# tomoyoshki/focal

Hardware: AMD Instinct MI355X
Metric: pretrain windows/sec (whole node), FOCAL SW_Transformer (higher is better)
Workload: dtype bf16

## Files before the change

focal_amd/csrc/gemm_dw_group.hpp:

```cpp
#pragma once
#include "gemm_pipe.hpp"

constexpr int DWG_MAX_PROBLEMS = FOCAL_DW_GROUP_MAX_PROBLEMS;

struct DwGroupProblem {
  const bf16_t* A; const bf16_t* B; float* C; float* colsum;
  int lda, ldb, ldc;
  int M, N, rows;
  int splits;
  int exclusive;
};
struct DwGroupParams {
  int nprob;
  int wg_end[DWG_MAX_PROBLEMS];
  DwGroupProblem prob[DWG_MAX_PROBLEMS];
};

template <int RPS, int NST>
__global__ __launch_bounds__(512) void focal_dw_group_kernel(const DwGroupParams gp) {
  constexpr int SUB_BYTES = RPS * 128;
  constexpr int STAGE_BYTES = 4 * SUB_BYTES;
  constexpr int PPS = RPS / 8;
  constexpr int LPW = 4 * PPS / 8;
  static_assert(RPS % 32 == 0 && (4 * PPS) % 8 == 0, "stage geometry");
  constexpr int NFA = 4, NFB = 2;
  constexpr int WPITCH = 32 + 4;
  static_assert(NST * STAGE_BYTES >= 8 * 16 * WPITCH * 4, "epilogue staging must fit in the ring");
  extern __shared__ __attribute__((aligned(1024))) char dwg_lds[];
  const int tid = threadIdx.x, lane = tid & 63, g = lane >> 4, l15 = lane & 15, tq = l15 >> 2, tp = l15 & 3;
  const int wave = __builtin_amdgcn_readfirstlane(tid >> 6);
  const int wm = wave >> 2, wn = wave & 3;

  const int logical = xcd_remap(blockIdx.x, gridDim.x);
  int pi = 0;
#pragma unroll
  for (int q = 0; q < DWG_MAX_PROBLEMS - 1; ++q) pi += (q < gp.nprob - 1 && logical >= gp.wg_end[q]) ? 1 : 0;
  const DwGroupProblem& p = gp.prob[pi];
  const int local = logical - (pi > 0 ? gp.wg_end[pi - 1] : 0);
  const int tiles_n = p.N >> 7, ntiles = (p.M >> 7) * tiles_n;
  const int tile = local % ntiles, sp = local / ntiles;
  const int m0 = (tile / tiles_n) << 7, n0 = (tile % tiles_n) << 7;
  const int KT = p.rows / RPS;
  const int kt_per = (KT + p.splits - 1) / p.splits;
  const int kt0 = min(KT, sp * kt_per), kt1 = min(KT, kt0 + kt_per);
  const int nk = kt1 - kt0;

  auto swz = [](int r) { return (((r >> 1) & 1) << 1) | (((r >> 3) & 1) << 2); };

  uint32_t goff[LPW];
  const char* gbase[LPW];
  long gstep[LPW];
#pragma unroll
  for (int t = 0; t < LPW; ++t) {
    const int q = wave + 8 * t;
    const int sub = q / PPS, row = 8 * (q % PPS) + (lane >> 3), pos = lane & 7;
    const int chunk = pos ^ swz(row);
    if (sub < 2) {
      goff[t] = (uint32_t)(((long)row * p.lda + m0 + 64 * sub + chunk * 8) * 2);
      gbase[t] = reinterpret_cast<const char*>(p.A);
      gstep[t] = (long)RPS * p.lda * 2;
    } else {
      goff[t] = (uint32_t)(((long)row * p.ldb + n0 + 64 * (sub - 2) + chunk * 8) * 2);
      gbase[t] = reinterpret_cast<const char*>(p.B);
      gstep[t] = (long)RPS * p.ldb * 2;
    }
  }
  auto fill = [&](int kt, int stage) {
#pragma unroll
    for (int t = 0; t < LPW; ++t) {
      const int q = wave + 8 * t;
      char* dst = dwg_lds + stage * STAGE_BYTES + q * 1024;
      __builtin_amdgcn_global_load_lds((pipe_glb_ptr)(gbase[t] + (long)kt * gstep[t] + goff[t]), (pipe_lds_ptr)dst, 16, 0, 0);
    }
  };

  f32x4 acc[NFA][NFB], accb[NFA];
#pragma unroll
  for (int i = 0; i < NFA; ++i) {
    accb[i] = f32x4{0.f, 0.f, 0.f, 0.f};
#pragma unroll
    for (int j = 0; j < NFB; ++j) acc[i][j] = f32x4{0.f, 0.f, 0.f, 0.f};
  }
  const bool do_bias = (p.colsum != nullptr) && (n0 == 0) && (wn == 0);
  bf16x8 ones;
#pragma unroll
  for (int e = 0; e < 8; ++e) ones[e] = (bf16_t)1.0f;

  const int row_lo = 8 * g + tq;
  const int sw = swz(row_lo);
  int fr_a[NFA], fr_b[NFB];
#pragma unroll
  for (int i = 0; i < NFA; ++i) fr_a[i] = wm * SUB_BYTES + row_lo * 128 + (((2 * i + (tp >> 1)) ^ sw) << 4) + (tp & 1) * 8;
#pragma unroll
  for (int j = 0; j < NFB; ++j)
    fr_b[j] = (2 + (wn >> 1)) * SUB_BYTES + row_lo * 128 + (((2 * (2 * (wn & 1) + j) + (tp >> 1)) ^ sw) << 4) + (tp & 1) * 8;
  const uint32_t lds0 = pipe_lds_addr(dwg_lds);
  auto compute = [&](int stage) {
    const uint32_t sb = lds0 + stage * STAGE_BYTES;
    pipe_static_for<0, RPS / 32>([&](auto kc) {
      constexpr int KO = decltype(kc)::value * 32 * 128;
      bf16x4 al[NFA], ah[NFA], bl[NFB], bh[NFB];
#pragma unroll
      for (int i = 0; i < NFA; ++i) {
        al[i] = pipe_lds_read_tr<KO>(sb + fr_a[i]);
        ah[i] = pipe_lds_read_tr<KO + 4 * 128>(sb + fr_a[i]);
      }
#pragma unroll
      for (int j = 0; j < NFB; ++j) {
        bl[j] = pipe_lds_read_tr<KO>(sb + fr_b[j]);
        bh[j] = pipe_lds_read_tr<KO + 4 * 128>(sb + fr_b[j]);
      }
      bf16x8 xa[NFA], wb[NFB];
#pragma unroll
      for (int i = 0; i < NFA; ++i) xa[i] = __builtin_shufflevector(al[i], ah[i], 0, 1, 2, 3, 4, 5, 6, 7);
#pragma unroll
      for (int j = 0; j < NFB; ++j) wb[j] = __builtin_shufflevector(bl[j], bh[j], 0, 1, 2, 3, 4, 5, 6, 7);
      pipe_lds_wait(xa, wb);
#pragma unroll
      for (int i = 0; i < NFA; ++i)
#pragma unroll
        for (int j = 0; j < NFB; ++j) acc[i][j] = mma16(wb[j], xa[i], acc[i][j]);
      if (do_bias) {
#pragma unroll
        for (int i = 0; i < NFA; ++i) accb[i] = mma16(ones, xa[i], accb[i]);
      }
    });
  };

#pragma unroll
  for (int s = 0; s < NST - 1; ++s)
    if (s < nk) fill(kt0 + s, s);
  int stage = 0, fstage = NST - 1;
  for (int i = 0; i < nk; ++i) {
    const int ahead = nk - 1 - i;
    if (NST >= 4 && ahead >= 2) pipe_wait_barrier<2 * LPW>();
    else if (NST >= 3 && ahead >= 1) pipe_wait_barrier<LPW>();
    else pipe_wait_barrier<0>();
    if (i + NST - 1 < nk) fill(kt0 + i + NST - 1, fstage);
    compute(stage);
    stage = (stage + 1 == NST) ? 0 : stage + 1;
    fstage = (fstage + 1 == NST) ? 0 : fstage + 1;
  }
  if (nk == 0) return;
#if defined(DWG_LAB_NOEPI)
  {
    float lab = 0.f;
#pragma unroll
    for (int i = 0; i < NFA; ++i) {
      lab += accb[i][0];
#pragma unroll
      for (int j = 0; j < NFB; ++j) lab += acc[i][j][0] + acc[i][j][1] + acc[i][j][2] + acc[i][j][3];
    }
    if (lab == 12345.678f) p.C[0] = 1.f;
    return;
  }
#endif

  const int mrow = m0 + 64 * wm, ncol = n0 + 32 * wn;
  if (p.splits == 1 && p.exclusive) {
#pragma unroll
    for (int i = 0; i < NFA; ++i)
#pragma unroll
      for (int j = 0; j < NFB; ++j) {
        float4* dst = reinterpret_cast<float4*>(p.C + (long)(mrow + 16 * i + l15) * p.ldc + ncol + 16 * j + 4 * g);
        float4 v = *dst;
        v.x += acc[i][j][0]; v.y += acc[i][j][1]; v.z += acc[i][j][2]; v.w += acc[i][j][3];
        *dst = v;
      }
  } else {
    asm volatile("s_barrier" ::: "memory");
    float* est = reinterpret_cast<float*>(dwg_lds) + wave * 16 * WPITCH;
    const int ecol = lane & 31, erow = lane >> 5;
#pragma unroll
    for (int i = 0; i < NFA; ++i) {
#pragma unroll
      for (int j = 0; j < NFB; ++j)
        *reinterpret_cast<float4*>(est + l15 * WPITCH + j * 16 + g * 4) = make_float4(acc[i][j][0], acc[i][j][1], acc[i][j][2], acc[i][j][3]);
      asm volatile("s_waitcnt lgkmcnt(0)" ::: "memory");
      float* crow = p.C + (long)(mrow + 16 * i + erow) * p.ldc + ncol + ecol;
#pragma unroll 4
#if defined(DWG_LAB_STORE)
      for (int r = 0; r < 16; r += 2) crow[(long)r * p.ldc] = est[(r + erow) * WPITCH + ecol];
#else
      for (int r = 0; r < 16; r += 2) atomicAdd(crow + (long)r * p.ldc, est[(r + erow) * WPITCH + ecol]);
#endif
      asm volatile("s_waitcnt lgkmcnt(0)" ::: "memory");
    }
  }
  if (do_bias && g == 0) {
#pragma unroll
    for (int i = 0; i < NFA; ++i) atomicAdd(p.colsum + mrow + 16 * i + l15, accb[i][0]);
  }
}

template <int RPS>
static inline int focal_dw_group_plan(DwGroupParams& gp, int target_wgs, int min_steps) {
  long work = 0;
  for (int q = 0; q < gp.nprob; ++q) work += (long)(gp.prob[q].M >> 7) * (gp.prob[q].N >> 7) * (gp.prob[q].rows / RPS);
  long per = (work + target_wgs - 1) / target_wgs;
  if (per < min_steps) per = min_steps;
  int total = 0;
  for (int it = 0; it < 64; ++it) {
    total = 0;
    for (int q = 0; q < gp.nprob; ++q) {
      DwGroupProblem& p = gp.prob[q];
      const int KT = p.rows / RPS;
      int s = (int)((KT + per - 1) / per);
      if (s < 1) s = 1;
      p.splits = s;
      total += (p.M >> 7) * (p.N >> 7) * s;
    }
    bool can_shrink = false;
    for (int q = 0; q < gp.nprob; ++q) can_shrink = can_shrink || gp.prob[q].splits > 1;
    if (total <= target_wgs || !can_shrink) break;
    per += (per + 15) / 16;
  }
  int end = 0;
  for (int q = 0; q < gp.nprob; ++q) {
    end += (gp.prob[q].M >> 7) * (gp.prob[q].N >> 7) * gp.prob[q].splits;
    gp.wg_end[q] = end;
  }
  for (int q = gp.nprob; q < DWG_MAX_PROBLEMS; ++q) gp.wg_end[q] = end;
  return end;
}

template <int RPS, int NST>
static inline hipError_t focal_launch_dw_group(const DwGroupParams& gp, int wgs, hipStream_t stream) {
  constexpr int LDS_BYTES = NST * 4 * RPS * 128;
  auto kern = focal_dw_group_kernel<RPS, NST>;
  static std::atomic<bool> attr_set{false};
  if (!attr_set.load(std::memory_order_acquire)) {
    hipError_t e = hipFuncSetAttribute(reinterpret_cast<const void*>(kern), hipFuncAttributeMaxDynamicSharedMemorySize, LDS_BYTES);
    if (e != hipSuccess) return e;
    attr_set.store(true, std::memory_order_release);
  }
  FOCAL_LAUNCH(kern, dim3(wgs), dim3(512), LDS_BYTES, stream, gp);
  return hipGetLastError();
}
```

focal_amd/csrc/linear.hip:

```cpp
#include <stdlib.h>
#include "gemm.hpp"
#include "gemm_dw_group.hpp"
#include "gemm_dw_ring.hpp"
#include "gemm_ring.hpp"

static MaskParams to_mask(const focal_drop_desc& d, int ncols) {
  MaskParams m;
  m.seed = d.rng;
  m.stream_elem = d.stream_elem;
  m.p_elem = d.p_elem;
  m.stream_path = d.stream_path;
  m.p_path = d.p_path;
  m.rows_per_sample = d.rows_per_sample;
  m.ncols = ncols;
  return m;
}
static MaskParams no_mask() {
  MaskParams m;
  memset(&m, 0, sizeof(m));
  return m;
}

static int check_desc(const focal_linear_desc* d) {
  FOCAL_CHECK_ARG(d != nullptr, "linear: null descriptor");
// ... 134 lines not shown
  p.proB = no_mask();
  focal_drop_desc dd;
  memset(&dd, 0, sizeof(dd));
  if (mask) dd = *mask;
  p.epi = to_mask(dd, d->K);
  hipError_t e;
  if (d->K == 64 && d->M >= 4096 && !focal_ring_disabled() &&
      focal_ring_fits<float, EPI_LN_BWD, true, 128, 64, 6, true, 8, 1, 2, false>(p)) {
    focal_note_kernel("focal_gemm_ring_kernel<f32, epi=%d (LayerNorm backward), trB=1, 128x64, 8x1 waves, ring 6, panel resident>", EPI_LN_BWD);
    e = focal_launch_gemm_ring<float, EPI_LN_BWD, true, 128, 64, 6, true, 8, 1, 2, false>(p, (hipStream_t)stream);
  } else if (d->K == 128 && d->M >= 4096 && !focal_ring_disabled() &&
             focal_ring_fits<float, EPI_LN_BWD, true, 64, 128, 4, false, 4, 1, 2, false, false>(p)) {
    focal_note_kernel("focal_gemm_ring_kernel<f32, epi=%d (LayerNorm backward), trB=1, 64x128, 4x1 waves, ring 4>", EPI_LN_BWD);
    e = focal_launch_gemm_ring<float, EPI_LN_BWD, true, 64, 128, 4, false, 4, 1, 2, false, false>(p, (hipStream_t)stream);
  } else if (d->K == 256 && d->M >= 2048 && !focal_ring_disabled() && getenv("FOCAL_LAB_LN_BWD_RING256") != nullptr &&
             focal_ring_fits<float, EPI_LN_BWD, true, 64, 256, 2, false, 4, 1, 2, false, false>(p)) {
    focal_note_kernel("focal_gemm_ring_kernel<f32, epi=%d (LayerNorm backward), trB=1, 64x256, 4x1 waves, ring 2>", EPI_LN_BWD);
    e = focal_launch_gemm_ring<float, EPI_LN_BWD, true, 64, 256, 2, false, 4, 1, 2, false, false>(p, (hipStream_t)stream);
  } else {
    focal_note_kernel("focal_gemm_pipe_kernel<f32, epi=%d (LayerNorm backward), trB=1, %dx%d, 4x%d waves>", EPI_LN_BWD, d->K == 256 ? 64 : 128,
                      d->K, d->K == 256 ? 2 : 1);
    e = d->K == 64    ? focal_launch_gemm_pipe<float, EPI_LN_BWD, true, 128, 64, 2, 4, 1>(p, (hipStream_t)stream)
        : d->K == 128 ? focal_launch_gemm_pipe<float, EPI_LN_BWD, true, 128, 128, 2, 4, 1>(p, (hipStream_t)stream)
                      : focal_launch_gemm_pipe<float, EPI_LN_BWD, true, 64, 256, 2, 4, 2>(p, (hipStream_t)stream);
  }
  if (e != hipSuccess) {
    focal_set_error("linear_bwd_data_ln: launch failed: %s", hipGetErrorString(e));
    return FOCAL_EHIP;
  }
  return FOCAL_OK;
}

extern "C" int focal_linear_bwd_weight(const focal_linear_desc* d, const void* dy, const void* x, float* dw, float* dbias,
                                       void* stream) {
  if (int rc = check_desc(d)) return rc;
  FOCAL_CHECK_ARG(dy && x && dw, "linear_bwd_weight: null tensor");
  GemmSpec s;
  s.compute = d->dtype;
  s.a_dtype = d->y_dtype; s.b_dtype = d->x_dtype; s.c_dtype = FOCAL_F32;
  s.tra = true; s.trb = true;
  const bool masked = d->epilogue == FOCAL_EPI_RESIDUAL || (d->y_dtype == FOCAL_F32 && d->x_dtype != FOCAL_F32);
  s.proA = masked ? PRO_MASK : PRO_NONE;
  s.proB = PRO_NONE;
  s.epi = EPI_ATOMIC;
  GemmParams p;
  memset(&p, 0, sizeof(p));
  p.M = d->N; p.N = d->K; p.K = d->M;
  p.A = dy; p.lda = d->N;
  p.B = x; p.ldb = d->K;
  p.C = dw; p.ldc = d->K;
  p.batch = 1; p.alpha = 1.f;
  p.splits = 1;
  p.dw_target = d->dw_workgroups;
  p.proA = masked ? to_mask(d->out_drop, d->N) : no_mask();
  p.proB = no_mask();
  p.epi = no_mask();
  p.colsumA = dbias;
  return focal_launch_gemm(s, p, (hipStream_t)stream);
}

static bool dw_launch_plan(const focal_linear_desc* d, int* kernel, int* wgs) {
  if (check_desc(d) != FOCAL_OK) return false;
  int bm, bn, splits;
  focal_dw_plan(d->N, d->K, d->M, d->dw_workgroups, &bm, &bn, &splits);
  const bool masked = d->epilogue == FOCAL_EPI_RESIDUAL || (d->y_dtype == FOCAL_F32 && d->x_dtype != FOCAL_F32);
  const bool ring = d->dtype == FOCAL_BF16 && d->x_dtype == FOCAL_BF16 && d->y_dtype == FOCAL_BF16 && !masked && bm == 64 && bn == 64 &&
                    focal_dw_ring_shape(d->N, d->K, d->M);
  *kernel = ring ? 2 : 1;
  if (ring && splits >= 2) splits = focal_dw_ring_pairs(d->N, d->K, splits);
  *wgs = ((d->N + bm - 1) / bm) * ((d->K + bn - 1) / bn) * splits;
  return true;
}

extern "C" int focal_linear_bwd_weight_workgroups(const focal_linear_desc* d) {
  int kernel, wgs;
  return dw_launch_plan(d, &kernel, &wgs) ? wgs : 0;
}

extern "C" int focal_linear_bwd_weight_kernel(const focal_linear_desc* d) {
  int kernel, wgs;
  return dw_launch_plan(d, &kernel, &wgs) ? kernel : 0;
}

static bool dw_group_fits(const focal_dw_problem& q) {
  return q.M > 0 && q.N > 0 && q.K > 0 && q.M % 64 == 0 && q.N % 128 == 0 && q.K % 128 == 0 && q.dy && q.x && q.dw &&
         ((uintptr_t)q.dy % 16 == 0) && ((uintptr_t)q.x % 16 == 0) && ((uintptr_t)q.dw % 16 == 0);
}

extern "C" int focal_linear_bwd_weight_group_supported(int dtype, int M, int N, int K) {
  return dtype == FOCAL_BF16 && M > 0 && M % 64 == 0 && N % 128 == 0 && K % 128 == 0;
}

static int dw_group_build(int dtype, int n, const focal_dw_problem* probs, DwGroupParams* gp, int* wgs) {
  FOCAL_CHECK_ARG(dtype == FOCAL_BF16, "linear_bwd_weight_group: bf16 operands only (dtype %d)", dtype);
  FOCAL_CHECK_ARG(n >= 1 && n <= DWG_MAX_PROBLEMS && probs, "linear_bwd_weight_group: 1 .. %d problems (got %d)", DWG_MAX_PROBLEMS, n);
  memset(gp, 0, sizeof(*gp));
  gp->nprob = n;
  for (int i = 0; i < n; ++i) {
    const focal_dw_problem& q = probs[i];
    FOCAL_CHECK_ARG(dw_group_fits(q), "linear_bwd_weight_group: problem %d (M=%d N=%d K=%d) needs M %% 64 == 0, N, K %% 128 == 0 and 16-byte aligned tensors", i, q.M, q.N, q.K);
    DwGroupProblem& p = gp->prob[i];
    p.A = reinterpret_cast<const bf16_t*>(q.dy); p.lda = q.N;
    p.B = reinterpret_cast<const bf16_t*>(q.x); p.ldb = q.K;
    p.C = q.dw; p.ldc = q.K;
    p.colsum = q.dbias;
    p.M = q.N; p.N = q.K; p.rows = q.M;
    p.exclusive = q.exclusive ? 1 : 0;
  }
  const int target = getenv("FOCAL_LAB_DWG_TARGET") ? atoi(getenv("FOCAL_LAB_DWG_TARGET")) : 256, min_steps = 8;
  *wgs = focal_dw_group_plan<64>(*gp, target, min_steps);
  return FOCAL_OK;
}

static bool dw_ring_group_fits(const focal_dw_problem& q) {
  return q.M >= 64 && q.M % 64 == 0 && q.N > 0 && q.N % 64 == 0 && q.K > 0 && q.K % 64 == 0 && q.dy && q.x && q.dw &&
         ((uintptr_t)q.dy % 16 == 0) && ((uintptr_t)q.x % 16 == 0);
}
static bool dw_group_uses_ring(int n, const focal_dw_problem* probs) {
  if (!probs || n < 1 || n > DWR_MAX_PROBLEMS) return false;
  bool all128 = true, all64 = true;
  for (int i = 0; i < n; ++i) { all128 = all128 && dw_group_fits(probs[i]); all64 = all64 && dw_ring_group_fits(probs[i]); }
  return !all128 && all64;
}
static int dw_ring_group_build(int dtype, int n, const focal_dw_problem* probs, DwRingGroupParams* gp, int* wgs) {
  FOCAL_CHECK_ARG(dtype == FOCAL_BF16, "linear_bwd_weight_group: bf16 operands only (dtype %d)", dtype);
  memset(gp, 0, sizeof(*gp));
  gp->nprob = n;
  for (int i = 0; i < n; ++i) {
    const focal_dw_problem& q = probs[i];
    GemmParams& p = gp->prob[i];
    p.M = q.N; p.N = q.K; p.K = q.M;
    p.A = q.dy; p.lda = q.N;
    p.B = q.x; p.ldb = q.K;
    p.C = q.dw; p.ldc = q.K;
    p.batch = 1; p.alpha = 1.f; p.splits = 1;
    p.colsumA = q.dbias;
  }
  *wgs = focal_dw_ring_group_plan<2>(*gp);
  return FOCAL_OK;
}

extern "C" int focal_linear_bwd_weight_group_kind(int dtype, int M, int N, int K) {
  if (dtype != FOCAL_BF16 || M <= 0 || M % 64 != 0) return 0;
  if (N % 128 == 0 && K % 128 == 0) return 2;
  return (N > 0 && K > 0 && N % 64 == 0 && K % 64 == 0) ? 1 : 0;
}

extern "C" int focal_linear_bwd_weight_group(int dtype, int n, const focal_dw_problem* probs, void* stream) {
  if (dw_group_uses_ring(n, probs)) {
    DwRingGroupParams rp;
    int rw = 0;
    if (int rc = dw_ring_group_build(dtype, n, probs, &rp, &rw)) return rc;
    focal_note_kernel("focal_dw_ring_group_kernel<64, 4, 2>");
    hipError_t e = focal_launch_dw_ring_group<64, 4, 2>(rp, rw, (hipStream_t)stream);
    if (e != hipSuccess) {
      focal_set_error("linear_bwd_weight_group (64-tile ring): launch failed: %s", hipGetErrorString(e));
      return FOCAL_EHIP;
    }
    return FOCAL_OK;
  }
  DwGroupParams gp;
  int wgs = 0;
  if (int rc = dw_group_build(dtype, n, probs, &gp, &wgs)) return rc;
  hipError_t e = focal_launch_dw_group<64, 4>(gp, wgs, (hipStream_t)stream);
  if (e != hipSuccess) {
    focal_set_error("linear_bwd_weight_group: launch failed: %s", hipGetErrorString(e));
    return FOCAL_EHIP;
  }
  return FOCAL_OK;
}

static int dw_tail_build(int compute, int n, const focal_dw_problem* probs, int workgroups, DwTailGroup* g) {
  FOCAL_CHECK_ARG(compute == FOCAL_BF16 || compute == FOCAL_F32, "linear_bwd_weight_group_f32: bad compute dtype %d", compute);
  FOCAL_CHECK_ARG(n >= 1 && n <= DW_TAIL_MAX && probs, "linear_bwd_weight_group_f32: 1 .. %d problems (got %d)", DW_TAIL_MAX, n);
  memset(g, 0, sizeof(*g));
  g->n = n;
  const int target = (workgroups > 0 ? workgroups : 1024) / n;
  int end = 0;
  for (int i = 0; i < n; ++i) {
    const focal_dw_problem& q = probs[i];
    FOCAL_CHECK_ARG(q.dy && q.x && q.dw && q.M > 0 && q.N > 0 && q.K > 0, "linear_bwd_weight_group_f32: problem %d: null tensor or empty shape", i);
    GemmParams& p = g->p[i];
    p.M = q.N; p.N = q.K; p.K = q.M;
    p.A = q.dy; p.lda = q.N;
    p.B = q.x; p.ldb = q.K;
    p.C = q.dw; p.ldc = q.K;
    p.batch = 1; p.alpha = 1.f;
    p.colsumA = q.dbias;
    int bm, bn, splits;
    focal_dw_plan(p.M, p.N, q.M, target < 1 ? 1 : target, &bm, &bn, &splits);
    p.splits = splits;
    end += ((p.M + bm - 1) / bm) * ((p.N + bn - 1) / bn) * splits;
    g->wg_end[i] = end;
  }
// ... 24 lines not shown
```

focal_amd/ops.py:

```python
import ctypes as C
import math
import os

import torch

from . import _lib
from ._lib import (ACT_GELU, ACT_NONE, ACT_RELU_OUT, EPI_GELU, EPI_NONE, EPI_RELU, EPI_RESIDUAL, FOCAL_BF16, FOCAL_F32,
                   AdamWDesc, AttnDesc, BNDesc, ConvDesc, ConvInDesc, DropDesc, Embed2Desc, EmbedDesc, FFTDesc, GRUDesc, LinearDesc,
                   LNDesc, LossDesc, MlpDesc, check)

_TORCH2CODE = {torch.float32: FOCAL_F32, torch.bfloat16: FOCAL_BF16}
_CODE2TORCH = {v: k for k, v in _TORCH2CODE.items()}


def code(dtype):
    return _TORCH2CODE[dtype]


def torch_dtype(c):
    return _CODE2TORCH[c]


def _stream():
    return torch.cuda.current_stream().cuda_stream
# ... 444 lines not shown
    out = torch.empty(rows, Cc, dtype=dtype, device=g.device)
    check(_lib.load().focal_mask_cast(code(dtype), rows, Cc, _p(g), C.byref(mask or NO_DROP), _p(out), _stream()))
    return out


def linear_desc(dtype_code, M, N, K, x_dtype, y_dtype, act_in=ACT_NONE, epilogue=EPI_NONE, splits=1, out_drop=None, dw_workgroups=0):
    return LinearDesc(dtype_code, M, N, K, x_dtype, y_dtype, act_in, epilogue, splits, out_drop or NO_DROP, dw_workgroups)


def linear_fwd(d, x, w, bias, resid, y, act_grad=None):
    check(_lib.load().focal_linear_fwd(C.byref(d), _p(x), _p(w), _p(bias), _p(resid), _p(y), _p(act_grad), _stream()))


def linear_resid_ln_fwd(d, x, w, bias, resid, y, gamma, beta, out_dtype, eps=1e-5):
    y_ln = torch.empty(d.M, d.N, dtype=out_dtype, device=y.device)
    stats = torch.empty(d.M, 2, dtype=torch.float32, device=y.device)
    check(_lib.load().focal_linear_resid_ln_fwd(C.byref(d), _p(x), _p(w), _p(bias), _p(resid), _p(y), _p(gamma), _p(beta), eps,
                                                _p(y_ln), _p(stats), _stream()))
    return y_ln, stats


def resid_ln_supported(dtype_code, N, K):
    return bool(_lib.load().focal_linear_resid_ln_supported(dtype_code, N, K))


def linear_bwd_data(d, dy, w, x, dx):
    check(_lib.load().focal_linear_bwd_data(C.byref(d), _p(dy), _p(w), _p(x), _p(dx), _stream()))


def bwd_data_ln_supported(dtype_code, N, K):
    return bool(_lib.load().focal_linear_bwd_data_ln_supported(dtype_code, N, K))


def linear_bwd_data_ln(d, dy, w, ln_x, ln_stats, ln_gamma, g, dgamma, dbeta, g_masked=None, mask=None):
    _need_cuda(dy, w, ln_x, ln_stats, ln_gamma, g, dgamma, dbeta, g_masked)
    if g_masked is not None:
        mask = mask or NO_DROP
    check(_lib.load().focal_linear_bwd_data_ln(C.byref(d), _p(dy), _p(w), _p(ln_x), _p(ln_stats), _p(ln_gamma), _p(g), _p(dgamma), _p(dbeta),
                                               _p(g_masked), C.byref(mask) if mask is not None else None, _stream()))


def linear_bwd_weight(d, dy, x, dw, dbias):
    check(_lib.load().focal_linear_bwd_weight(C.byref(d), _p(dy), _p(x), _p(dw), _p(dbias), _stream()))


def dw_group_supported(dtype_code, M, N, K):
    return bool(_lib.load().focal_linear_bwd_weight_group_supported(dtype_code, M, N, K))


def dw_group_kind(dtype_code, M, N, K):
    return int(_lib.load().focal_linear_bwd_weight_group_kind(dtype_code, M, N, K))


def _dw_problems(items, exclusive):
    arr = (_lib.DwProblem * len(items))()
    for i, (dy, x, dw, db) in enumerate(items):
        _need_cuda(dy, x, dw, db)
        arr[i] = _lib.DwProblem(_p(dy), _p(x), _p(dw), _p(db), dy.shape[0], dy.shape[1], x.shape[1], 1 if exclusive else 0)
    return arr


DW_GROUP_MAX_PROBLEMS = 20


def linear_bwd_weight_group(dtype_code, items, exclusive=True):
    arr = _dw_problems(items, exclusive)
    check(_lib.load().focal_linear_bwd_weight_group(dtype_code, len(items), arr, _stream()))


DW_TAIL_MAX = 8


def linear_bwd_weight_group_f32(compute_code, items, workgroups=0):
    for dy, x, dw, db in items:
        if dy.dtype != torch.float32 or x.dtype != torch.float32 or dy.dim() != 2 or x.dim() != 2 or not (dy.is_contiguous() and x.is_contiguous()):
            raise _lib.FocalHipError("linear_bwd_weight_group_f32: dy and x must be contiguous fp32 matrices")
    check(_lib.load().focal_linear_bwd_weight_group_f32(compute_code, len(items), _dw_problems(items, False), workgroups, _stream()))


def linear_bwd_weight_group_workgroups(dtype_code, items, exclusive=True):
    return _lib.load().focal_linear_bwd_weight_group_workgroups(dtype_code, len(items), _dw_problems(items, exclusive))


def linear(x, w, bias=None, *, compute, y_dtype=None, resid=None, act_in=ACT_NONE, epilogue=EPI_NONE, splits=1,
           out_drop=None, act_grad=None):
    _need_cuda(x, w, bias, resid)
    M, K = x.shape
    N = w.shape[0]
    y_dtype = y_dtype or compute
    d = linear_desc(code(compute), M, N, K, code(x.dtype), code(y_dtype), act_in, epilogue, splits, out_drop)
    y = (torch.zeros if splits > 1 else torch.empty)(M, N, dtype=y_dtype, device=x.device)
    linear_fwd(d, x, w, bias, resid, y, act_grad)
    return y, d


def mlp_supported(dtype, Cc, hidden):
    return bool(_lib.load().focal_mlp_supported(code(dtype), Cc, hidden))


def mlp_desc(dtype_code, M, Cc, hidden, drop_hidden=None, drop_out=None, ln_eps=1e-5):
    return MlpDesc(dtype_code, M, Cc, hidden, drop_hidden or NO_DROP, drop_out or NO_DROP, ln_eps)


def mlp_mask_bits(d, device):
    if d.drop_hidden.p_elem <= 0.0:
        return None
    return torch.empty(d.M, 8, dtype=torch.int32, device=device)


def _next_ln(d, like, next_ln):
    if next_ln is None:
        return (None,) * 4, None
    y_ln = torch.empty(d.M, d.C, dtype=like.dtype, device=like.device)
    stats = torch.empty(d.M, 2, dtype=torch.float32, device=like.device)
    return (_p(next_ln[0]), _p(next_ln[1]), _p(y_ln), _p(stats)), (y_ln, stats)


def _ln_mask(ln, key):
    return None if ln is None else C.byref(ln.get(key) or NO_DROP)


def mlp_fwd(d, a, resid, w1, b1, w2, b2, y, next_ln=None, mask_bits=None):
    _need_cuda(a, resid, w1, b1, w2, b2, y, mask_bits)
    ln_ptrs, out = _next_ln(d, a, next_ln)
    check(_lib.load().focal_mlp_fwd(C.byref(d), _p(a), _p(resid), _p(w1), _p(b1), _p(w2), _p(b2), _p(y), *ln_ptrs, _p(mask_bits), _stream()))
    return out


def mlp_proj_supported(dtype, Cc, hidden):
    return bool(_lib.load().focal_mlp_proj_supported(code(dtype), Cc, hidden))


def mlp_proj_fwd(d, o, x, wp, bp, drop_proj, g2, bt2, x_mid, w1, b1, w2, b2, y, next_ln=None, mask_bits=None):
    _need_cuda(o, x, wp, bp, g2, bt2, x_mid, w1, b1, w2, b2, y, mask_bits)
    a2 = torch.empty(d.M, d.C, dtype=o.dtype, device=o.device)
    st2 = torch.empty(d.M, 2, dtype=torch.float32, device=o.device)
    mask = drop_proj or NO_DROP
    ln_ptrs, out = _next_ln(d, o, next_ln)
    check(_lib.load().focal_mlp_proj_fwd(C.byref(d), _p(o), _p(x), _p(wp), _p(bp), C.byref(mask), _p(g2), _p(bt2), _p(x_mid), _p(a2), _p(st2), _p(w1), _p(b1),
                                         _p(w2), _p(b2), _p(y), *ln_ptrs, _p(mask_bits), _stream()))
    return (a2, st2), out


def mlp_wide_supported(dtype, Cc, hidden):
    return bool(_lib.load().focal_mlp_wide_supported(code(dtype), Cc, hidden))


def mlp_wide_fwd(d, a, resid, w1, b1, w2, b2, y, h, hg, next_ln=None):
    _need_cuda(a, resid, w1, b1, w2, b2, y, h, hg)
    assert h.shape == (d.M, d.hidden) and hg.shape == h.shape and h.dtype == a.dtype and hg.dtype == a.dtype and h.is_contiguous() and hg.is_contiguous()
    ln_ptrs, out = _next_ln(d, a, next_ln)
    check(_lib.load().focal_mlp_wide_fwd(C.byref(d), _p(a), _p(resid), _p(w1), _p(b1), _p(w2), _p(b2), _p(y), _p(h), _p(hg), *ln_ptrs, _stream()))
    return out


def mlp_wide_proj_supported(dtype, Cc, hidden):
    return bool(_lib.load().focal_mlp_wide_proj_supported(code(dtype), Cc, hidden))


def mlp_wide_proj_fwd(d, o, x, wp, bp, drop_proj, g2, bt2, x_mid, w1, b1, w2, b2, y, h, hg, next_ln=None):
    _need_cuda(o, x, wp, bp, g2, bt2, x_mid, w1, b1, w2, b2, y, h, hg)
    a2 = torch.empty(d.M, d.C, dtype=o.dtype, device=o.device)
    st2 = torch.empty(d.M, 2, dtype=torch.float32, device=o.device)
    mask = drop_proj or NO_DROP
    ln_ptrs, out = _next_ln(d, o, next_ln)
    check(_lib.load().focal_mlp_wide_proj_fwd(C.byref(d), _p(o), _p(x), _p(wp), _p(bp), C.byref(mask), _p(g2), _p(bt2), _p(x_mid), _p(a2), _p(st2), _p(w1), _p(b1),
# ... 477 lines not shown
```

Measured before the change: 52580.

## Balance grouped weight-gradient GEMM work with a stream-K style unit split

Replaces the per-problem split-K planner of the grouped dW kernel with a work-unit scheduler. Each workgroup can now walk several (tile, k-range) segments in a loop, so the total (tile, stage) units are spread evenly across workgroups. A host-side cost model picks between this balanced cut and the old sliced cut, and memoizes the choice per shape. The epilogue now stages the whole 64x32 wave tile at once and rotates the atomic row order by segment key to spread atomic contention. The balanced cut adds per-segment atomic flushes and barriers in exchange for less tail imbalance.

```diff
diff --git a/focal_amd/csrc/gemm_dw_group.hpp b/focal_amd/csrc/gemm_dw_group.hpp
--- a/focal_amd/csrc/gemm_dw_group.hpp
+++ b/focal_amd/csrc/gemm_dw_group.hpp
@@ -1,4 +1,5 @@
 #pragma once
+#include <climits>
 #include "gemm_pipe.hpp"
 
 constexpr int DWG_MAX_PROBLEMS = FOCAL_DW_GROUP_MAX_PROBLEMS;
@@ -7,14 +8,51 @@
   const bf16_t* A; const bf16_t* B; float* C; float* colsum;
   int lda, ldb, ldc;
   int M, N, rows;
-  int splits;
+  int band, nfull;
   int exclusive;
 };
 struct DwGroupParams {
   int nprob;
-  int wg_end[DWG_MAX_PROBLEMS];
+  int pieces;
+  int share, extra;
+  int chunk_end[2 * DWG_MAX_PROBLEMS];
   DwGroupProblem prob[DWG_MAX_PROBLEMS];
 };
+static_assert(sizeof(DwGroupParams) <= 4096, "the kernel-argument struct must stay within what a launch accepts");
+
+struct DwGroupSeg {
+  int prob, tile, kt0, nk;
+  int adv;
+  int key;
+  int whole;
+};
+
+template <int RPS>
+__host__ __device__ __forceinline__ DwGroupSeg focal_dw_group_locate(const DwGroupParams& gp, int u, int u1) {
+  int ci = 0, start = 0;
+#pragma unroll
+  for (int q = 0; q < 2 * DWG_MAX_PROBLEMS - 1; ++q) {
+    const int e = gp.chunk_end[q];
+    if (u >= e) { ci = q + 1; start = e; }
+  }
+  const bool rem = ci >= gp.nprob;
+  DwGroupSeg s;
+  s.prob = rem ? ci - gp.nprob : ci;
+  const DwGroupProblem& p = gp.prob[s.prob];
+  const int ntiles = (p.M >> 7) * (p.N >> 7), KT = p.rows / RPS;
+  const int base = p.nfull * p.band;
+  const int len = rem ? KT - base : p.band;
+  const int local = u - start;
+  const int piece = gp.pieces ? local : local / len, within = gp.pieces ? 0 : local - piece * len;
+  const int bandi = rem ? p.nfull : piece / ntiles;
+  s.tile = rem ? piece : piece - bandi * ntiles;
+  s.kt0 = (rem ? base : bandi * p.band) + within;
+  s.nk = (gp.pieces || len - within < u1 - u) ? len - within : u1 - u;
+  s.adv = gp.pieces ? 1 : s.nk;
+  s.key = 2 * bandi + (within != 0 ? 1 : 0);
+  s.whole = (s.kt0 == 0 && s.nk == KT) ? 1 : 0;
+  return s;
+}
 
 template <int RPS, int NST>
 __global__ __launch_bounds__(512) void focal_dw_group_kernel(const DwGroupParams gp) {
@@ -25,66 +63,13 @@
   static_assert(RPS % 32 == 0 && (4 * PPS) % 8 == 0, "stage geometry");
   constexpr int NFA = 4, NFB = 2;
   constexpr int WPITCH = 32 + 4;
-  static_assert(NST * STAGE_BYTES >= 8 * 16 * WPITCH * 4, "epilogue staging must fit in the ring");
+  static_assert(NST * STAGE_BYTES >= 8 * 64 * WPITCH * 4, "epilogue staging (a wave's 64 x 32 outputs, eight waves) must fit in the ring");
   extern __shared__ __attribute__((aligned(1024))) char dwg_lds[];
   const int tid = threadIdx.x, lane = tid & 63, g = lane >> 4, l15 = lane & 15, tq = l15 >> 2, tp = l15 & 3;
   const int wave = __builtin_amdgcn_readfirstlane(tid >> 6);
   const int wm = wave >> 2, wn = wave & 3;
 
-  const int logical = xcd_remap(blockIdx.x, gridDim.x);
-  int pi = 0;
-#pragma unroll
-  for (int q = 0; q < DWG_MAX_PROBLEMS - 1; ++q) pi += (q < gp.nprob - 1 && logical >= gp.wg_end[q]) ? 1 : 0;
-  const DwGroupProblem& p = gp.prob[pi];
-  const int local = logical - (pi > 0 ? gp.wg_end[pi - 1] : 0);
-  const int tiles_n = p.N >> 7, ntiles = (p.M >> 7) * tiles_n;
-  const int tile = local % ntiles, sp = local / ntiles;
-  const int m0 = (tile / tiles_n) << 7, n0 = (tile % tiles_n) << 7;
-  const int KT = p.rows / RPS;
-  const int kt_per = (KT + p.splits - 1) / p.splits;
-  const int kt0 = min(KT, sp * kt_per), kt1 = min(KT, kt0 + kt_per);
-  const int nk = kt1 - kt0;
-
   auto swz = [](int r) { return (((r >> 1) & 1) << 1) | (((r >> 3) & 1) << 2); };
-
-  uint32_t goff[LPW];
-  const char* gbase[LPW];
-  long gstep[LPW];
-#pragma unroll
-  for (int t = 0; t < LPW; ++t) {
-    const int q = wave + 8 * t;
-    const int sub = q / PPS, row = 8 * (q % PPS) + (lane >> 3), pos = lane & 7;
-    const int chunk = pos ^ swz(row);
-    if (sub < 2) {
-      goff[t] = (uint32_t)(((long)row * p.lda + m0 + 64 * sub + chunk * 8) * 2);
-      gbase[t] = reinterpret_cast<const char*>(p.A);
-      gstep[t] = (long)RPS * p.lda * 2;
-    } else {
-      goff[t] = (uint32_t)(((long)row * p.ldb + n0 + 64 * (sub - 2) + chunk * 8) * 2);
-      gbase[t] = reinterpret_cast<const char*>(p.B);
-      gstep[t] = (long)RPS * p.ldb * 2;
-    }
-  }
-  auto fill = [&](int kt, int stage) {
-#pragma unroll
-    for (int t = 0; t < LPW; ++t) {
-      const int q = wave + 8 * t;
-      char* dst = dwg_lds + stage * STAGE_BYTES + q * 1024;
-      __builtin_amdgcn_global_load_lds((pipe_glb_ptr)(gbase[t] + (long)kt * gstep[t] + goff[t]), (pipe_lds_ptr)dst, 16, 0, 0);
-    }
-  };
-
-  f32x4 acc[NFA][NFB], accb[NFA];
-#pragma unroll
-  for (int i = 0; i < NFA; ++i) {
-    accb[i] = f32x4{0.f, 0.f, 0.f, 0.f};
-#pragma unroll
-    for (int j = 0; j < NFB; ++j) acc[i][j] = f32x4{0.f, 0.f, 0.f, 0.f};
-  }
-  const bool do_bias = (p.colsum != nullptr) && (n0 == 0) && (wn == 0);
-  bf16x8 ones;
-#pragma unroll
-  for (int e = 0; e < 8; ++e) ones[e] = (bf16_t)1.0f;
 
   const int row_lo = 8 * g + tq;
   const int sw = swz(row_lo);
@@ -95,133 +80,293 @@
   for (int j = 0; j < NFB; ++j)
     fr_b[j] = (2 + (wn >> 1)) * SUB_BYTES + row_lo * 128 + (((2 * (2 * (wn & 1) + j) + (tp >> 1)) ^ sw) << 4) + (tp & 1) * 8;
   const uint32_t lds0 = pipe_lds_addr(dwg_lds);
-  auto compute = [&](int stage) {
-    const uint32_t sb = lds0 + stage * STAGE_BYTES;
-    pipe_static_for<0, RPS / 32>([&](auto kc) {
-      constexpr int KO = decltype(kc)::value * 32 * 128;
-      bf16x4 al[NFA], ah[NFA], bl[NFB], bh[NFB];
+  bf16x8 ones;
+#pragma unroll
+  for (int e = 0; e < 8; ++e) ones[e] = (bf16_t)1.0f;
+
+  const int logical = xcd_remap(blockIdx.x, gridDim.x);
+  int u = logical * gp.share + min(logical, gp.extra);
+  const int u1 = u + gp.share + (logical < gp.extra ? 1 : 0);
+
+  while (u < u1) {
+    const DwGroupSeg seg = focal_dw_group_locate<RPS>(gp, u, u1);
+    const DwGroupProblem& p = gp.prob[seg.prob];
+    const int tiles_n = p.N >> 7;
+    const int m0 = (seg.tile / tiles_n) << 7, n0 = (seg.tile % tiles_n) << 7;
+    const int kt0 = seg.kt0, nk = seg.nk;
+
+    uint32_t goff[LPW];
+    const char* gbase[LPW];
+    long gstep[LPW];
+#pragma unroll
+    for (int t = 0; t < LPW; ++t) {
+      const int q = wave + 8 * t;
+      const int sub = q / PPS, row = 8 * (q % PPS) + (lane >> 3), pos = lane & 7;
+      const int chunk = pos ^ swz(row);
+      if (sub < 2) {
+        goff[t] = (uint32_t)(((long)row * p.lda + m0 + 64 * sub + chunk * 8) * 2);
+        gbase[t] = reinterpret_cast<const char*>(p.A);
+        gstep[t] = (long)RPS * p.lda * 2;
+      } else {
+        goff[t] = (uint32_t)(((long)row * p.ldb + n0 + 64 * (sub - 2) + chunk * 8) * 2);
+        gbase[t] = reinterpret_cast<const char*>(p.B);
+        gstep[t] = (long)RPS * p.ldb * 2;
+      }
+    }
+    auto fill = [&](int kt, int stage) {
+#pragma unroll
+      for (int t = 0; t < LPW; ++t) {
+        const int q = wave + 8 * t;
+        char* dst = dwg_lds + stage * STAGE_BYTES + q * 1024;
+        __builtin_amdgcn_global_load_lds((pipe_glb_ptr)(gbase[t] + (long)kt * gstep[t] + goff[t]), (pipe_lds_ptr)dst, 16, 0, 0);
+      }
+    };
+
+    f32x4 acc[NFA][NFB], accb[NFA];
+#pragma unroll
+    for (int i = 0; i < NFA; ++i) {
+      accb[i] = f32x4{0.f, 0.f, 0.f, 0.f};
+#pragma unroll
+      for (int j = 0; j < NFB; ++j) acc[i][j] = f32x4{0.f, 0.f, 0.f, 0.f};
+    }
+    const bool do_bias = (p.colsum != nullptr) && (n0 == 0) && (wn == 0);
+
+    auto compute = [&](int stage) {
+      const uint32_t sb = lds0 + stage * STAGE_BYTES;
+      pipe_static_for<0, RPS / 32>([&](auto kc) {
+        constexpr int KO = decltype(kc)::value * 32 * 128;
+        bf16x4 al[NFA], ah[NFA], bl[NFB], bh[NFB];
+#pragma unroll
+        for (int i = 0; i < NFA; ++i) {
+          al[i] = pipe_lds_read_tr<KO>(sb + fr_a[i]);
+          ah[i] = pipe_lds_read_tr<KO + 4 * 128>(sb + fr_a[i]);
+        }
+#pragma unroll
+        for (int j = 0; j < NFB; ++j) {
+          bl[j] = pipe_lds_read_tr<KO>(sb + fr_b[j]);
+          bh[j] = pipe_lds_read_tr<KO + 4 * 128>(sb + fr_b[j]);
+        }
+        bf16x8 xa[NFA], wb[NFB];
+#pragma unroll
+        for (int i = 0; i < NFA; ++i) xa[i] = __builtin_shufflevector(al[i], ah[i], 0, 1, 2, 3, 4, 5, 6, 7);
+#pragma unroll
+        for (int j = 0; j < NFB; ++j) wb[j] = __builtin_shufflevector(bl[j], bh[j], 0, 1, 2, 3, 4, 5, 6, 7);
+        pipe_lds_wait(xa, wb);
+#pragma unroll
+        for (int i = 0; i < NFA; ++i)
+#pragma unroll
+          for (int j = 0; j < NFB; ++j) acc[i][j] = mma16(wb[j], xa[i], acc[i][j]);
+        if (do_bias) {
+#pragma unroll
+          for (int i = 0; i < NFA; ++i) accb[i] = mma16(ones, xa[i], accb[i]);
+        }
+      });
+    };
+
+#pragma unroll
+    for (int s = 0; s < NST - 1; ++s)
+      if (s < nk) fill(kt0 + s, s);
+    int stage = 0, fstage = NST - 1;
+    for (int i = 0; i < nk; ++i) {
+      const int ahead = nk - 1 - i;
+      if (NST >= 4 && ahead >= 2) pipe_wait_barrier<2 * LPW>();
+      else if (NST >= 3 && ahead >= 1) pipe_wait_barrier<LPW>();
+      else pipe_wait_barrier<0>();
+      if (i + NST - 1 < nk) fill(kt0 + i + NST - 1, fstage);
+      compute(stage);
+      stage = (stage + 1 == NST) ? 0 : stage + 1;
+      fstage = (fstage + 1 == NST) ? 0 : fstage + 1;
+    }
+
+    const int mrow = m0 + 64 * wm, ncol = n0 + 32 * wn;
+#if defined(DWG_LAB_NOEPI)
+    {
+      float lab = 0.f;
 #pragma unroll
       for (int i = 0; i < NFA; ++i) {
-        al[i] = pipe_lds_read_tr<KO>(sb + fr_a[i]);
-        ah[i] = pipe_lds_read_tr<KO + 4 * 128>(sb + fr_a[i]);
-      }
-#pragma unroll
-      for (int j = 0; j < NFB; ++j) {
-        bl[j] = pipe_lds_read_tr<KO>(sb + fr_b[j]);
-        bh[j] = pipe_lds_read_tr<KO + 4 * 128>(sb + fr_b[j]);
-      }
-      bf16x8 xa[NFA], wb[NFB];
-#pragma unroll
-      for (int i = 0; i < NFA; ++i) xa[i] = __builtin_shufflevector(al[i], ah[i], 0, 1, 2, 3, 4, 5, 6, 7);
-#pragma unroll
-      for (int j = 0; j < NFB; ++j) wb[j] = __builtin_shufflevector(bl[j], bh[j], 0, 1, 2, 3, 4, 5, 6, 7);
-      pipe_lds_wait(xa, wb);
+        lab += accb[i][0];
+#pragma unroll
+        for (int j = 0; j < NFB; ++j) lab += acc[i][j][0] + acc[i][j][1] + acc[i][j][2] + acc[i][j][3];
+      }
+      if (lab == 12345.678f) p.C[0] = 1.f;
+    }
+#else
+    if (seg.whole && p.exclusive) {
 #pragma unroll
       for (int i = 0; i < NFA; ++i)
 #pragma unroll
-        for (int j = 0; j < NFB; ++j) acc[i][j] = mma16(wb[j], xa[i], acc[i][j]);
-      if (do_bias) {
-#pragma unroll
-        for (int i = 0; i < NFA; ++i) accb[i] = mma16(ones, xa[i], accb[i]);
-      }
-    });
-  };
-
-#pragma unroll
-  for (int s = 0; s < NST - 1; ++s)
-    if (s < nk) fill(kt0 + s, s);
-  int stage = 0, fstage = NST - 1;
-  for (int i = 0; i < nk; ++i) {
-    const int ahead = nk - 1 - i;
-    if (NST >= 4 && ahead >= 2) pipe_wait_barrier<2 * LPW>();
-    else if (NST >= 3 && ahead >= 1) pipe_wait_barrier<LPW>();
-    else pipe_wait_barrier<0>();
-    if (i + NST - 1 < nk) fill(kt0 + i + NST - 1, fstage);
-    compute(stage);
-    stage = (stage + 1 == NST) ? 0 : stage + 1;
-    fstage = (fstage + 1 == NST) ? 0 : fstage + 1;
-  }
-  if (nk == 0) return;
-#if defined(DWG_LAB_NOEPI)
-  {
-    float lab = 0.f;
-#pragma unroll
-    for (int i = 0; i < NFA; ++i) {
-      lab += accb[i][0];
-#pragma unroll
-      for (int j = 0; j < NFB; ++j) lab += acc[i][j][0] + acc[i][j][1] + acc[i][j][2] + acc[i][j][3];
-    }
-    if (lab == 12345.678f) p.C[0] = 1.f;
-    return;
-  }
+        for (int j = 0; j < NFB; ++j) {
+          float4* dst = reinterpret_cast<float4*>(p.C + (long)(mrow + 16 * i + l15) * p.ldc + ncol + 16 * j + 4 * g);
+          float4 v = *dst;
+          v.x += acc[i][j][0]; v.y += acc[i][j][1]; v.z += acc[i][j][2]; v.w += acc[i][j][3];
+          *dst = v;
+        }
+    } else {
+      asm volatile("s_barrier" ::: "memory");
+      float* est = reinterpret_cast<float*>(dwg_lds) + wave * 64 * WPITCH;
+#pragma unroll
+      for (int i = 0; i < NFA; ++i)
+#pragma unroll
+        for (int j = 0; j < NFB; ++j)
+          *reinterpret_cast<float4*>(est + (16 * i + l15) * WPITCH + j * 16 + g * 4) = make_float4(acc[i][j][0], acc[i][j][1], acc[i][j][2], acc[i][j][3]);
+      asm volatile("s_waitcnt lgkmcnt(0)" ::: "memory");
+      const int ecol = lane & 31, erow = lane >> 5;
+      float* c0 = p.C + (long)mrow * p.ldc + ncol + ecol;
+      const int rp0 = (seg.key * 5) & 31;
+#pragma unroll 4
+      for (int k = 0; k < 32; ++k) {
+        const int row = 2 * ((k + rp0) & 31) + erow;
+#if defined(DWG_LAB_STORE)
+        c0[(long)row * p.ldc] = est[row * WPITCH + ecol];
+#else
+        atomicAdd(c0 + (long)row * p.ldc, est[row * WPITCH + ecol]);
 #endif
-
-  const int mrow = m0 + 64 * wm, ncol = n0 + 32 * wn;
-  if (p.splits == 1 && p.exclusive) {
-#pragma unroll
-    for (int i = 0; i < NFA; ++i)
-#pragma unroll
-      for (int j = 0; j < NFB; ++j) {
-        float4* dst = reinterpret_cast<float4*>(p.C + (long)(mrow + 16 * i + l15) * p.ldc + ncol + 16 * j + 4 * g);
-        float4 v = *dst;
-        v.x += acc[i][j][0]; v.y += acc[i][j][1]; v.z += acc[i][j][2]; v.w += acc[i][j][3];
-        *dst = v;
-      }
-  } else {
-    asm volatile("s_barrier" ::: "memory");
-    float* est = reinterpret_cast<float*>(dwg_lds) + wave * 16 * WPITCH;
-    const int ecol = lane & 31, erow = lane >> 5;
-#pragma unroll
-    for (int i = 0; i < NFA; ++i) {
-#pragma unroll
-      for (int j = 0; j < NFB; ++j)
-        *reinterpret_cast<float4*>(est + l15 * WPITCH + j * 16 + g * 4) = make_float4(acc[i][j][0], acc[i][j][1], acc[i][j][2], acc[i][j][3]);
-      asm volatile("s_waitcnt lgkmcnt(0)" ::: "memory");
-      float* crow = p.C + (long)(mrow + 16 * i + erow) * p.ldc + ncol + ecol;
-#pragma unroll 4
-#if defined(DWG_LAB_STORE)
-      for (int r = 0; r < 16; r += 2) crow[(long)r * p.ldc] = est[(r + erow) * WPITCH + ecol];
-#else
-      for (int r = 0; r < 16; r += 2) atomicAdd(crow + (long)r * p.ldc, est[(r + erow) * WPITCH + ecol]);
+      }
+    }
+    if (do_bias && g == 0) {
+#pragma unroll
+      for (int i = 0; i < NFA; ++i) atomicAdd(p.colsum + mrow + 16 * i + l15, accb[i][0]);
+    }
 #endif
-      asm volatile("s_waitcnt lgkmcnt(0)" ::: "memory");
-    }
-  }
-  if (do_bias && g == 0) {
-#pragma unroll
-    for (int i = 0; i < NFA; ++i) atomicAdd(p.colsum + mrow + 16 * i + l15, accb[i][0]);
-  }
-}
-
-template <int RPS>
-static inline int focal_dw_group_plan(DwGroupParams& gp, int target_wgs, int min_steps) {
-  long work = 0;
-  for (int q = 0; q < gp.nprob; ++q) work += (long)(gp.prob[q].M >> 7) * (gp.prob[q].N >> 7) * (gp.prob[q].rows / RPS);
-  long per = (work + target_wgs - 1) / target_wgs;
+    u += seg.adv;
+    if (u < u1) asm volatile("s_waitcnt lgkmcnt(0)\n\ts_barrier" ::: "memory");
+  }
+}
+
+static inline void focal_dw_group_chunks(DwGroupParams& gp, int RPS) {
+  long long end = 0;
+  for (int q = 0; q < gp.nprob; ++q) {
+    const DwGroupProblem& p = gp.prob[q];
+    end += (long long)(p.M >> 7) * (p.N >> 7) * p.nfull * (gp.pieces ? 1 : p.band);
+    gp.chunk_end[q] = (int)end;
+  }
+  for (int q = 0; q < gp.nprob; ++q) {
+    const DwGroupProblem& p = gp.prob[q];
+    const int rem = p.rows / RPS - p.nfull * p.band;
+    end += (long long)(p.M >> 7) * (p.N >> 7) * (gp.pieces ? (rem > 0 ? 1 : 0) : rem);
+    gp.chunk_end[gp.nprob + q] = (int)end;
+  }
+  for (int q = 2 * gp.nprob; q < 2 * DWG_MAX_PROBLEMS; ++q) gp.chunk_end[q] = (int)end;
+}
+
+template <int RPS>
+static inline int focal_dw_group_plan_balanced(DwGroupParams& gp, long long units, long long tiles, int target_wgs, int min_steps) {
+  long long G = units / min_steps;
+  if (G < tiles) G = tiles;
+  if (G > target_wgs) G = target_wgs;
+  if (G > units) G = units;
+  const long long band = (units + G - 1) / G;
+  G = (units + band - 1) / band;
+  gp.pieces = 0;
+  gp.share = (int)(units / G);
+  gp.extra = (int)(units % G);
+  for (int q = 0; q < gp.nprob; ++q) {
+    gp.prob[q].band = (int)band;
+    gp.prob[q].nfull = (int)((gp.prob[q].rows / RPS) / band);
+  }
+  focal_dw_group_chunks(gp, RPS);
+  return (int)G;
+}
+
+template <int RPS>
+static inline int focal_dw_group_plan_sliced(DwGroupParams& gp, long long units, int target_wgs, int min_steps) {
+  long long per = (units + target_wgs - 1) / target_wgs;
   if (per < min_steps) per = min_steps;
-  int total = 0;
   for (int it = 0; it < 64; ++it) {
-    total = 0;
+    long long total = 0;
+    bool can_shrink = false;
     for (int q = 0; q < gp.nprob; ++q) {
       DwGroupProblem& p = gp.prob[q];
       const int KT = p.rows / RPS;
-      int s = (int)((KT + per - 1) / per);
-      if (s < 1) s = 1;
-      p.splits = s;
-      total += (p.M >> 7) * (p.N >> 7) * s;
-    }
-    bool can_shrink = false;
-    for (int q = 0; q < gp.nprob; ++q) can_shrink = can_shrink || gp.prob[q].splits > 1;
+      int sl = (int)((KT + per - 1) / per);
+      if (sl < 1) sl = 1;
+      p.band = (KT + sl - 1) / sl;
+      p.nfull = KT / p.band;
+      total += (long long)(p.M >> 7) * (p.N >> 7) * sl;
+      can_shrink = can_shrink || sl > 1;
+    }
     if (total <= target_wgs || !can_shrink) break;
     per += (per + 15) / 16;
   }
-  int end = 0;
+  gp.pieces = 1;
+  gp.share = 1;
+  gp.extra = 0;
+  focal_dw_group_chunks(gp, RPS);
+  return gp.chunk_end[2 * DWG_MAX_PROBLEMS - 1];
+}
+
+constexpr int DWG_FLUSH_STAGES = 5;
+enum { DWG_CUT_AUTO = 0, DWG_CUT_BALANCED = 1, DWG_CUT_SLICED = 2 };
+
+template <int RPS>
+static inline int focal_dw_group_plan(DwGroupParams& gp, int target_wgs, int min_steps, int cut = DWG_CUT_AUTO, int* chosen = nullptr) {
+  long long units = 0, tiles = 0;
   for (int q = 0; q < gp.nprob; ++q) {
-    end += (gp.prob[q].M >> 7) * (gp.prob[q].N >> 7) * gp.prob[q].splits;
-    gp.wg_end[q] = end;
-  }
-  for (int q = gp.nprob; q < DWG_MAX_PROBLEMS; ++q) gp.wg_end[q] = end;
-  return end;
+    const long long t = (long long)(gp.prob[q].M >> 7) * (gp.prob[q].N >> 7);
+    tiles += t;
+    units += t * (gp.prob[q].rows / RPS);
+  }
+  if (units < 1 || units > INT_MAX) return -1;
+  if (target_wgs < 1) target_wgs = 1;
+  if (min_steps < 1) min_steps = 1;
+  int wgs = 0;
+  struct Memo { unsigned long long key; int cut; };
+  static thread_local Memo memo[16] = {};
+  static thread_local int memo_next = 0;
+  unsigned long long key = 1469598103934665603ull;
+  if (cut == DWG_CUT_AUTO) {
+    auto mix = [&key](long long v) { key = (key ^ (unsigned long long)v) * 1099511628211ull; };
+    mix(gp.nprob); mix(target_wgs); mix(min_steps);
+    for (int q = 0; q < gp.nprob; ++q) { mix(gp.prob[q].M); mix(gp.prob[q].N); mix(gp.prob[q].rows); }
+    key |= 1;
+    for (const Memo& m : memo)
+      if (m.key == key) cut = m.cut;
+  }
+  if (cut == DWG_CUT_AUTO) {
+    wgs = focal_dw_group_plan_balanced<RPS>(gp, units, tiles, target_wgs, min_steps);
+    long long cost_b = 0;
+    for (int w = 0; w < wgs; ++w) {
+      int u = w * gp.share + (w < gp.extra ? w : gp.extra), segs = 0;
+      const int u1 = u + gp.share + (w < gp.extra ? 1 : 0);
+      for (; u < u1; ++segs) u += focal_dw_group_locate<RPS>(gp, u, u1).adv;
+      const long long c = gp.share + (w < gp.extra ? 1 : 0) + (long long)DWG_FLUSH_STAGES * segs;
+      if (c > cost_b) cost_b = c;
+    }
+    wgs = focal_dw_group_plan_sliced<RPS>(gp, units, target_wgs, min_steps);
+    long long cost_s = 0;
+    for (int q = 0; q < gp.nprob; ++q) cost_s = gp.prob[q].band > cost_s ? gp.prob[q].band : cost_s;
+    cost_s = (cost_s + DWG_FLUSH_STAGES) * ((wgs + target_wgs - 1) / target_wgs);
+    cut = cost_b < cost_s ? DWG_CUT_BALANCED : DWG_CUT_SLICED;
+    memo[memo_next] = Memo{key, cut};
+    memo_next = (memo_next + 1) & 15;
+    if (cut == DWG_CUT_BALANCED) wgs = focal_dw_group_plan_balanced<RPS>(gp, units, tiles, target_wgs, min_steps);
+  } else if (cut == DWG_CUT_BALANCED) {
+    wgs = focal_dw_group_plan_balanced<RPS>(gp, units, tiles, target_wgs, min_steps);
+  } else {
+    wgs = focal_dw_group_plan_sliced<RPS>(gp, units, target_wgs, min_steps);
+  }
+  if (chosen) *chosen = cut;
+  return wgs;
+}
+
+template <int RPS>
+static inline int focal_dw_group_segments(const DwGroupParams& gp, int wgs, int cap, int* out) {
+  int n = 0;
+  for (int w = 0; w < wgs; ++w) {
+    int u = w * gp.share + (w < gp.extra ? w : gp.extra);
+    const int u1 = u + gp.share + (w < gp.extra ? 1 : 0);
+    while (u < u1) {
+      const DwGroupSeg s = focal_dw_group_locate<RPS>(gp, u, u1);
+      if (n < cap && out) {
+        int* r = out + 6 * (long)n;
+        r[0] = w; r[1] = s.prob; r[2] = s.tile; r[3] = s.kt0; r[4] = s.nk;
+        r[5] = (s.whole && gp.prob[s.prob].exclusive) ? 1 : 0;
+      }
+      ++n;
+      u += s.adv;
+    }
+  }
+  return n;
 }
 
 template <int RPS, int NST>
diff --git a/focal_amd/csrc/linear.hip b/focal_amd/csrc/linear.hip
--- a/focal_amd/csrc/linear.hip
+++ b/focal_amd/csrc/linear.hip
@@ -240,8 +240,11 @@
   return dw_launch_plan(d, &kernel, &wgs) ? kernel : 0;
 }
 
+static bool dw_group_shape_fits(const focal_dw_problem& q) {
+  return q.M > 0 && q.N > 0 && q.K > 0 && q.M % 64 == 0 && q.N % 128 == 0 && q.K % 128 == 0;
+}
 static bool dw_group_fits(const focal_dw_problem& q) {
-  return q.M > 0 && q.N > 0 && q.K > 0 && q.M % 64 == 0 && q.N % 128 == 0 && q.K % 128 == 0 && q.dy && q.x && q.dw &&
+  return dw_group_shape_fits(q) && q.dy && q.x && q.dw &&
          ((uintptr_t)q.dy % 16 == 0) && ((uintptr_t)q.x % 16 == 0) && ((uintptr_t)q.dw % 16 == 0);
 }
 
@@ -249,14 +252,15 @@
   return dtype == FOCAL_BF16 && M > 0 && M % 64 == 0 && N % 128 == 0 && K % 128 == 0;
 }
 
-static int dw_group_build(int dtype, int n, const focal_dw_problem* probs, DwGroupParams* gp, int* wgs) {
+static int dw_group_build(int dtype, int n, const focal_dw_problem* probs, DwGroupParams* gp, int* wgs, int target = 0, int min_steps = 0, int cut = 0,
+                          int* chosen = nullptr, bool tensors = true) {
   FOCAL_CHECK_ARG(dtype == FOCAL_BF16, "linear_bwd_weight_group: bf16 operands only (dtype %d)", dtype);
   FOCAL_CHECK_ARG(n >= 1 && n <= DWG_MAX_PROBLEMS && probs, "linear_bwd_weight_group: 1 .. %d problems (got %d)", DWG_MAX_PROBLEMS, n);
   memset(gp, 0, sizeof(*gp));
   gp->nprob = n;
   for (int i = 0; i < n; ++i) {
     const focal_dw_problem& q = probs[i];
-    FOCAL_CHECK_ARG(dw_group_fits(q), "linear_bwd_weight_group: problem %d (M=%d N=%d K=%d) needs M %% 64 == 0, N, K %% 128 == 0 and 16-byte aligned tensors", i, q.M, q.N, q.K);
+    FOCAL_CHECK_ARG(tensors ? dw_group_fits(q) : dw_group_shape_fits(q), "linear_bwd_weight_group: problem %d (M=%d N=%d K=%d) needs M %% 64 == 0, N, K %% 128 == 0 and 16-byte aligned tensors", i, q.M, q.N, q.K);
     DwGroupProblem& p = gp->prob[i];
     p.A = reinterpret_cast<const bf16_t*>(q.dy); p.lda = q.N;
     p.B = reinterpret_cast<const bf16_t*>(q.x); p.ldb = q.K;
@@ -265,9 +269,21 @@
     p.M = q.N; p.N = q.K; p.rows = q.M;
     p.exclusive = q.exclusive ? 1 : 0;
   }
-  const int target = getenv("FOCAL_LAB_DWG_TARGET") ? atoi(getenv("FOCAL_LAB_DWG_TARGET")) : 256, min_steps = 8;
-  *wgs = focal_dw_group_plan<64>(*gp, target, min_steps);
-  return FOCAL_OK;
+  if (target <= 0) target = getenv("FOCAL_LAB_DWG_TARGET") ? atoi(getenv("FOCAL_LAB_DWG_TARGET")) : 256;
+  if (min_steps <= 0) min_steps = 8;
+  if (cut <= 0 && getenv("FOCAL_LAB_DWG_CUT")) cut = atoi(getenv("FOCAL_LAB_DWG_CUT"));
+  FOCAL_CHECK_ARG(cut >= DWG_CUT_AUTO && cut <= DWG_CUT_SLICED, "linear_bwd_weight_group: cut %d (0 = by cost, 1 = balanced, 2 = sliced)", cut);
+  *wgs = focal_dw_group_plan<64>(*gp, target, min_steps, cut, chosen);
+  FOCAL_CHECK_ARG(*wgs > 0, "linear_bwd_weight_group: %d problems hold more than 2^31 - 1 (tile, stage) units", n);
+  return FOCAL_OK;
+}
+
+extern "C" int focal_dw_group_cut(int n, const focal_dw_problem* probs, int target, int min_steps, int cut, int cap, int* segs, int* info) {
+  DwGroupParams gp;
+  int wgs = 0, chosen = 0;
+  if (dw_group_build(FOCAL_BF16, n, probs, &gp, &wgs, target, min_steps, cut, &chosen, false) != FOCAL_OK) return -1;
+  if (info) { info[0] = wgs; info[1] = chosen; }
+  return focal_dw_group_segments<64>(gp, wgs, cap, segs);
 }
 
 static bool dw_ring_group_fits(const focal_dw_problem& q) {
diff --git a/focal_amd/ops.py b/focal_amd/ops.py
--- a/focal_amd/ops.py
+++ b/focal_amd/ops.py
@@ -550,6 +550,23 @@
     return _lib.load().focal_linear_bwd_weight_group_workgroups(dtype_code, len(items), _dw_problems(items, exclusive))
 
 
+def dw_group_cut(shapes, target=0, min_steps=0, cut=0):
+    lib = _lib.load()
+    fn = lib.focal_dw_group_cut
+    fn.restype = C.c_int
+    fn.argtypes = [C.c_int, C.POINTER(_lib.DwProblem), C.c_int, C.c_int, C.c_int, C.c_int, C.POINTER(C.c_int), C.POINTER(C.c_int)]
+    arr = (_lib.DwProblem * len(shapes))()
+    for i, (rows, N, K, exclusive) in enumerate(shapes):
+        arr[i] = _lib.DwProblem(None, None, None, None, rows, N, K, 1 if exclusive else 0)
+    info = (C.c_int * 2)()
+    n = fn(len(shapes), arr, target, min_steps, cut, 0, None, info)
+    if n < 0:
+        check(-1)
+    buf = (C.c_int * (6 * n))()
+    fn(len(shapes), arr, target, min_steps, cut, n, buf, info)
+    return info[0], info[1], [tuple(buf[6 * i:6 * i + 6]) for i in range(n)]
+
+
 def linear(x, w, bias=None, *, compute, y_dtype=None, resid=None, act_in=ACT_NONE, epilogue=EPI_NONE, splits=1,
            out_drop=None, act_grad=None):
     _need_cuda(x, w, bias, resid)
```

Result: no change. 52310 (-0.5%).
